# jinhojsk515/spmm

Hardware: AMD Instinct MI355X
Metric: pretrain molecules/sec (higher is better)
Workload: dtype bf16; 1 GPU; SPMM pretrain step, text 12 layers (fusion at 6) + PV 6 layers, H=768, 12 heads, queue 36864, train mode (dropout 0.1), fwd+bwd+clip+AdamW+EMA; global_batch=128, seq_len=128, parallelism=dp1, schedule=eager launches on three HIP streams, packed text rows

## Files before the change

include/spmm_hip.h:

```cpp
#ifndef SPMM_HIP_H
#define SPMM_HIP_H

#include <stdint.h>

#ifdef __HIPCC__
#include <hip/hip_runtime.h>
typedef hipStream_t spmm_stream_t;
#else
typedef void* spmm_stream_t;
#endif

#ifdef __cplusplus
extern "C" {
#endif

int spmm_version(void);
const char* spmm_last_error(void);

#define SPMM_EPI_BF16 0
#define SPMM_EPI_GELU 1
#define SPMM_EPI_F32 2
#define SPMM_EPI_F32_ATOMIC 3
#define SPMM_EPI_GELU_GRAD 4
#define SPMM_EPI_F32_ACC 5
#define SPMM_EPI_GELU_DERIV 6
#define SPMM_EPI_MUL 7

#define SPMM_GEMM_AUTO 0
#define SPMM_GEMM_K128 1
#define SPMM_GEMM_K256x128 2
#define SPMM_GEMM_K256 3
#define SPMM_GEMM_K128PC 5
#define SPMM_GEMM_K256P8 8
#define SPMM_GEMM_K256P8_TILES 9
#define SPMM_GEMM_AUTO_TILES 16
int spmm_gemm_nt(const void* A, long lda, const void* W, long ldw, int M, int N, int K, int splits, const float* bias,
                 const float* div_ptr, float alpha, const void* R, long ldr, const void* G, long ldg, void* C, long ldc,
                 void* C2, long ldc2, int epi, float* colsum, int kernel, const int* M_dev, spmm_stream_t stream);
long spmm_gemm_tn_workspace_bytes(int M, int N, int K, int splits);
int spmm_gemm_tn_splits(int M, int N, int K, int kernel);
int spmm_gemm_tn(const void* A, long lda, const void* B, long ldb, int M, int N, int K, int splits, float alpha, float* C,
                 long ldc, float* workspace, int kernel, const int* M_dev, spmm_stream_t stream);
int spmm_gemm_tn_reduce(const float* ws, int ns, int N, int K, float* C, long ldc, spmm_stream_t stream);
int spmm_colsum_bf16(const void* x, long ld, int R, int C, float* out, const int* R_dev, spmm_stream_t stream);

int spmm_attn_fwd(const void* Q, long ldq, const void* K, long ldk, const void* V, long ldv, const int* kmask,
                  const int* kv_seq, const int* q_row0, const int* q_len, const int* kv_row0, const int* kv_len, void* O,
                  long ldo, float* LSE, int nseq, int nH, int Lq, int Lkv, int causal_from, int is_cross, float dropout_p,
                  const uint64_t* seed_ptr, uint64_t seed_salt, int q_off, int kv_off, spmm_stream_t stream);
int spmm_attn_bwd(const void* Q, long ldq, const void* K, long ldk, const void* V, long ldv, const int* kmask,
                  const int* kv_seq, const int* q_row0, const int* q_len, const int* kv_row0, const int* kv_len,
                  const void* O, long ldo, const float* LSE, const void* dO, long lddo, void* dQ,
                  long lddq, void* dK, long lddk, void* dV, long lddv, int nseq, int nH, int Lq, int Lkv, int causal_from,
                  int is_cross, float dropout_p, const uint64_t* seed_ptr, uint64_t seed_salt, int q_off, int kv_off, int d_mode,
                  float* Dbuf, spmm_stream_t stream);

int spmm_xattn_supported(int H, int nH, int Lq, int Lkv);
int spmm_xattn_pack_wo(const void* W, long ldw, void* out, int H, spmm_stream_t stream);
int spmm_xattn_fwd(const void* Q, long ldq, const void* K, long ldk, const void* V, long ldv, const int* kmask,
                   const int* kv_seq, const int* q_row0, const int* q_len, const int* kv_row0, const int* kv_len,
                   const void* WoF, const float* bo, const void* R, long ldr, const float* gamma, const float* beta, float eps,
                   void* Y, long ldy, void* Z, long ldz, float* mean, float* rstd, void* CTX, long ldc, float* LSE,
                   int nseq, int nH, int Lq, int Lkv, float attn_dropout_p, uint64_t salt_a, float hidden_dropout_p,
                   uint64_t salt_h, const uint64_t* seed_ptr, long row_base, spmm_stream_t stream);
int spmm_segment_sum_bf16(const void* src, const int* start, const int* list, void* out, int U, long W, spmm_stream_t stream);

int spmm_ln_fwd(const void* x, const void* res, const float* gamma, const float* beta, void* y, void* zout, float* mean,
                float* rstd, long rows, int H, float eps, float dropout_p, const uint64_t* seed_ptr, uint64_t salt,
                const int* rows_dev, spmm_stream_t stream);
int spmm_ln_fwd_r32(const void* x, const float* res32, const float* gamma, const float* beta, void* y, float* y32, void* zout,
                    float* mean, float* rstd, long rows, int H, float eps, float dropout_p, const uint64_t* seed_ptr,
                    uint64_t salt, spmm_stream_t stream);
int spmm_ln_bwd(const void* dy, const void* dy2, const void* z, const float* mean, const float* rstd, const float* gamma,
                void* dz, void* dx, float* dgamma, float* dbeta, long rows, int H, float dropout_p,
                const uint64_t* seed_ptr, uint64_t salt, int drop_on_dy, float* dxsum, const int* rows_dev,
                const float* beta_from_y, spmm_stream_t stream);

int spmm_embed_step_ln_fwd(const int* ids, int pos_index, const int* pos_ptr, const float* word, const float* pos, const float* type0,
                           const float* gamma, const float* beta, void* y, long rows, int H, float eps, spmm_stream_t stream);

int spmm_decode_attn(const void* q, long ldq, const void* K, const void* V, long seq_stride, long tok_stride, long head_stride, const int* anc,
                     int anc_ld, int kv_div, int group, void* out, long ldo, int R, int nH, int Lkv, float scale,
                     const int* t_ptr, const void* knew, const void* vnew, long ldn, const int* rowmap, spmm_stream_t stream);

int spmm_decode_xattn(const void* q, long ldq, const void* K, const void* V, long ldkv, const int* kv_seq, const int* kv_row0,
                      const int* kv_len, int group, void* out, long ldo, int R, int nH, int Lkv_max, float scale, spmm_stream_t stream);

int spmm_beam_step(const float* logits, long ldl, int N, int k, int V, int Lmax, int F, int t, const int* t_ptr, int t_off,
                   int* tokens, float* cur_p, float* fin_p, int* fin_len, int* fin_tok, int* fin_n, unsigned char* done,
                   int* anc, int anc_ld, int* ids_out, int* parent_out, int* n_done, const int* mol, const int* rowmap,
                   spmm_stream_t stream);

int spmm_beam_step_until(const float* logits, long ldl, int N, int k, int V, int Lmax, int F, int t, const int* t_ptr, int t_off,
                         int* tokens, float* cur_p, float* fin_p, int* fin_len, int* fin_tok, int* fin_n, unsigned char* done,
                         int* anc, int anc_ld, int* ids_out, int* parent_out, int* n_done, const int* mol, const int* rowmap,
                         int need, spmm_stream_t stream);

int spmm_beam_step_sampled(const float* logits, long ldl, int N, int k, int V, int Lmax, int F, int t, const int* t_ptr, int t_off,
                           int* tokens, float* cur_p, float* fin_p, int* fin_len, int* fin_tok, int* fin_n, unsigned char* done,
                           int* anc, int anc_ld, int* ids_out, int* parent_out, int* n_done, const int* mol, const int* rowmap,
                           const float* noise, long ldn, spmm_stream_t stream);

int spmm_gumbel_noise(const uint64_t* seed_ptr, uint64_t salt, int N, int k, int V, int Lmax, int t, const int* t_ptr, int t_off,
                      const int* mol, long mol_base, float* out, long ldo, spmm_stream_t stream);

int spmm_logit_warp(const float* lc, const float* lu, long ld, int R, int V, float w, float temperature, int top_k, float top_p,
                    int min_keep, float* out, long ldo, spmm_stream_t stream);

#define SPMM_SYNTAX_MASKED (-1e30f)
int spmm_smiles_mask(float* logits, float* logits2, long ld, int R, int V, const int* tokens, long tok_ld, int hist_rows, int k,
                     const int* mol, int Lmax, int t, const int* t_ptr, int t_off, int t_last, const int* table, int* state_out,
                     spmm_stream_t stream);

int spmm_kv_prefill(const void* K, const void* V, long ld, long src_rows, const int* row0, const int* len, const int* dst_row, int E,
                    void* Kc, void* Vc, int R, int nH, int Lmax, spmm_stream_t stream);

int spmm_embed_ln_fwd(int mode, const int* ids, const float* word, const float* pos, const float* type0, const float* pv_x,
// ... 83 lines not shown
```

spmm_amd/csrc/gemm.hip:

```cpp
#include "common.h"
#include "../../include/spmm_hip.h"

namespace {

constexpr int BM = 128, BN = 128, BK = 64;
constexpr int TILE_BYTES = BM * BK * 2;
constexpr int STAGE_BYTES = 2 * TILE_BYTES;

enum Epi { EPI_BF16 = 0, EPI_GELU = 1, EPI_F32 = 2, EPI_F32_ATOMIC = 3, EPI_GELU_GRAD = 4, EPI_F32_ACC = 5, EPI_GELU_DERIV = 6, EPI_MUL = 7 };
constexpr bool epi_is_bf16(int e) { return e == EPI_BF16 || e == EPI_GELU || e == EPI_GELU_GRAD || e == EPI_GELU_DERIV || e == EPI_MUL; }

struct GemmP {
  const bf16* A; long lda;
  const bf16* W; long ldw;
  int M, N, K;
  int ksplit;
  const float* bias;
  const float* div_ptr;
  float alpha;
  const bf16* R; long ldr;
  const bf16* G; long ldg;
  void* C; long ldc;
  bf16* C2; long ldc2;
  float* colsum;
// ... 589 lines not shown
  {
    const int b = blockIdx.x, q = nt >> 3, r = nt & 7, xcd = b & 7, i = b >> 3;
    if (i >= (xcd < r ? q + 1 : q)) return;
    t = (xcd < r ? xcd * (q + 1) : r * (q + 1) + (xcd - r) * q) + i;
  }
  int tile_m, tile_n;
  tile_of(t, ntm, ntn, p.order, tile_m, tile_n);
  const int m0 = tile_m * BM3, n0 = tile_n * BN3;
  const int nk = p.K / BK;

  f32x16 acc[2][2][2];
#pragma unroll
  for (int h = 0; h < 2; ++h)
#pragma unroll
    for (int i = 0; i < 2; ++i)
#pragma unroll
      for (int j = 0; j < 2; ++j)
#pragma unroll
        for (int r = 0; r < 16; ++r) acc[h][i][j][r] = 0.f;

#define STAGE3(kt_)                                                                           \
  do {                                                                                        \
    char* b_ = smem3 + ((kt_) & 1) * STAGE3_BYTES;                                            \
    stage2_dma(p.A, p.lda, m0, p.M, (kt_) * BK, b_, tid, 4);                                  \
    stage2_dma(p.W, p.ldw, n0, p.N, (kt_) * BK, b_ + T3_BYTES, tid, 4);                       \
  } while (0)

  STAGE3(0);
  for (int kt = 0; kt < nk; ++kt) {
    __syncthreads();
    if (kt + 1 < nk) STAGE3(kt + 1);
    const char* As = smem3 + (kt & 1) * STAGE3_BYTES;
    const char* Ws = As + T3_BYTES;
#pragma unroll
    for (int kk = 0; kk < 4; ++kk) {
      const int s = kk * 2 + (lane >> 5);
      bf16x8 af[4], wf[2];
#pragma unroll
      for (int i = 0; i < 4; ++i) {
        const int ar = wm * 128 + i * 32 + (lane & 31);
        af[i] = *(const bf16x8*)(As + ar * 128 + ((s ^ ((ar >> 1) & 7)) << 4));
      }
#pragma unroll
      for (int i = 0; i < 2; ++i) {
        const int wr = wn * 64 + i * 32 + (lane & 31);
        wf[i] = *(const bf16x8*)(Ws + wr * 128 + ((s ^ ((wr >> 1) & 7)) << 4));
      }
#pragma unroll
      for (int h = 0; h < 2; ++h)
#pragma unroll
        for (int ni = 0; ni < 2; ++ni)
#pragma unroll
          for (int mi = 0; mi < 2; ++mi)
            acc[h][ni][mi] = __builtin_amdgcn_mfma_f32_32x32x16_bf16(wf[ni], af[h * 2 + mi], acc[h][ni][mi], 0, 0, 0);
    }
  }
#undef STAGE3
  __syncthreads();
  char* wt = smem3 + wave * 16384;
  float cs_carry[8] = {0.f, 0.f, 0.f, 0.f, 0.f, 0.f, 0.f, 0.f};
#pragma unroll
  for (int h = 0; h < 2; ++h)
    epilogue_bf16<EPI>(p, acc[h], wt, m0 + wm * 128 + h * 64, n0 + wn * 64, lane, cs_carry, h == 1);
}

constexpr int P8_HT = 128 * BK * 2;
constexpr int P8_BUF = 4 * P8_HT;
constexpr int P8_LDS = 2 * P8_BUF;
constexpr int P8_XLDS = 8 * 4096;

template <int OFF>
__device__ __forceinline__ void p8_dsr(bf16x8& d, uint32_t addr) {
  asm volatile("ds_read_b128 %0, %1 offset:%2" : "=v"(d) : "v"(addr), "n"(OFF) : "memory");
}

struct P8Out { uint32_t d[4]; };
__device__ __forceinline__ uint32_t p8_pack2(float a, float b) {
  typedef __bf16 bf16x2 __attribute__((ext_vector_type(2)));
  bf16x2 v; v[0] = (bf16)a; v[1] = (bf16)b;
  return __builtin_bit_cast(uint32_t, v);
}
__device__ __forceinline__ float p8_lo(uint32_t w) { return __builtin_bit_cast(float, w << 16); }
__device__ __forceinline__ float p8_hi(uint32_t w) { return __builtin_bit_cast(float, w & 0xffff0000u); }
typedef uint32_t u32x2 __attribute__((ext_vector_type(2)));
typedef uint32_t u32x4 __attribute__((ext_vector_type(4)));
template <int OFF>
__device__ __forceinline__ void p8_dsw64(uint32_t addr, uint32_t a, uint32_t b) {
  u32x2 v = {a, b};
  asm volatile("ds_write_b64 %0, %1 offset:%2" :: "v"(addr), "v"(v), "n"(OFF) : "memory");
}
template <int OFF>
__device__ __forceinline__ void p8_dsr128u(u32x4& d, uint32_t addr) {
  asm volatile("ds_read_b128 %0, %1 offset:%2" : "=v"(d) : "v"(addr), "n"(OFF) : "memory");
}

template <int EPI, bool INTERIOR, bool HAS_EX, typename Hook>
__device__ __forceinline__ void p8_epilogue_blocks(const GemmP& p, f32x4 (&acc)[2][4][4], uint32_t xb ,
                                                   int m_base, int n_base, int lane, Hook hook) {
  float scale = p.alpha;
  if (p.div_ptr) scale /= *p.div_ptr;
  const int m = lane & 15, g = lane >> 4, r8 = lane >> 3, c16 = lane & 7;
  f32x4 b[4];
#pragma unroll
  for (int ni = 0; ni < 4; ++ni) b[ni] = f32x4{0.f, 0.f, 0.f, 0.f};
  if (p.bias) {
#pragma unroll
    for (int ni = 0; ni < 4; ++ni)
      if (INTERIOR || n_base + ni * 16 + 4 * g < p.N) b[ni] = *(const f32x4*)(p.bias + n_base + ni * 16 + 4 * g);
  }
  uint32_t wad[4];
#pragma unroll
  for (int ni = 0; ni < 4; ++ni) wad[ni] = xb + (uint32_t)(m * 128 + ((((ni * 2 + (g >> 1)) ^ (m & 7)) << 4) | ((g & 1) << 3)));
  const uint32_t rad = xb + (uint32_t)(r8 * 128 + ((c16 ^ (r8 & 7)) << 4));
  const long n = n_base + c16 * 8;
  const bool n_ok = INTERIOR || n < p.N;
  const long row0 = m_base + r8;
  bf16* cp = (bf16*)p.C + row0 * p.ldc + n;
  constexpr bool GELU2 = EPI == EPI_GELU || EPI == EPI_GELU_DERIV;
  constexpr bool DERIV = EPI == EPI_GELU_DERIV;
  constexpr bool MULG = EPI == EPI_MUL;
  bf16* c2p = GELU2 && p.C2 ? p.C2 + row0 * p.ldc2 + n : nullptr;
  u32x4 ex[8];
  const bf16* esrc = (EPI == EPI_GELU_GRAD || MULG) ? p.G : p.R;
  const long eld = (EPI == EPI_GELU_GRAD || MULG) ? p.ldg : p.ldr;
  const long nn = n_ok ? n : 0;
#define P8_EX_LOAD1(I_, R_)                                                                                            \
  do {                                                                                                                 \
    ex[I_] = *(const u32x4*)(esrc + (R_) * eld + nn);                                                                  \
  } while (0)
#define P8_LOAD_EX(H)                                                          \
  if constexpr (HAS_EX) {                                                      \
    _Pragma("unroll") for (int i_ = 0; i_ < 8; ++i_) {                         \
      long r_ = row0 + (H) * 64 + i_ * 8;                                      \
      if (!INTERIOR) r_ = r_ < p.M ? r_ : p.M - 1;                             \
      P8_EX_LOAD1(i_, r_);                                                     \
    }                                                                          \
  }
  P8_LOAD_EX(0);
  float cs[8] = {0.f, 0.f, 0.f, 0.f, 0.f, 0.f, 0.f, 0.f};
#pragma unroll
  for (int h = 0; h < 2; ++h)
#pragma unroll
    for (int mi = 0; mi < 4; ++mi) {
      const int blk = h * 4 + mi;
      const uint32_t bo = (blk & 1) * 2048;
      const bool ok1 = INTERIOR || (n_ok && row0 + blk * 16 < p.M), ok2 = INTERIOR || (n_ok && row0 + blk * 16 + 8 < p.M);
      float v[4][4];
#pragma unroll
      for (int ni = 0; ni < 4; ++ni)
#pragma unroll
        for (int j = 0; j < 4; ++j) v[ni][j] = acc[h][mi][ni][j] * scale + b[ni][j];
#pragma unroll
      for (int ni = 0; ni < 4; ++ni) acc[h][mi][ni] = f32x4{0.f, 0.f, 0.f, 0.f};
      u32x4 o1, o2;
      if constexpr (GELU2) {
        float w[4][4];
#pragma unroll
        for (int ni = 0; ni < 4; ++ni)
#pragma unroll
          for (int j = 0; j < 4; j += 2) {
            const f32x2 x = {v[ni][j], v[ni][j + 1]};
            f32x2 gg, dd = x;
            gelu_erf_pair<DERIV>(x, gg, dd);
            v[ni][j] = gg.x; v[ni][j + 1] = gg.y;
            w[ni][j] = dd.x; w[ni][j + 1] = dd.y;
          }
        if (c2p) {
          u32x4 q1, q2;
#pragma unroll
          for (int ni = 0; ni < 4; ++ni) p8_dsw64<0>(wad[ni] + bo, p8_pack2(w[ni][0], w[ni][1]), p8_pack2(w[ni][2], w[ni][3]));
#pragma unroll
          for (int ni = 0; ni < 4; ++ni) p8_dsw64<0>(wad[ni] + (bo ^ 2048u), p8_pack2(v[ni][0], v[ni][1]), p8_pack2(v[ni][2], v[ni][3]));
          p8_dsr128u<0>(q1, rad + bo);
          p8_dsr128u<1024>(q2, rad + bo);
          p8_dsr128u<0>(o1, rad + (bo ^ 2048u));
          p8_dsr128u<1024>(o2, rad + (bo ^ 2048u));
          asm volatile("s_waitcnt lgkmcnt(0)" ::: "memory");
          __builtin_amdgcn_sched_barrier(0);
          if (ok1) *(u32x4*)(c2p + (long)blk * 16 * p.ldc2) = q1;
          if (ok2) *(u32x4*)(c2p + (long)blk * 16 * p.ldc2 + 8 * p.ldc2) = q2;
        }
      }
      if (!(GELU2 && c2p)) {
#pragma unroll
        for (int ni = 0; ni < 4; ++ni) p8_dsw64<0>(wad[ni] + bo, p8_pack2(v[ni][0], v[ni][1]), p8_pack2(v[ni][2], v[ni][3]));
        p8_dsr128u<0>(o1, rad + bo);
        p8_dsr128u<1024>(o2, rad + bo);
        asm volatile("s_waitcnt lgkmcnt(0)" ::: "memory");
        __builtin_amdgcn_sched_barrier(0);
      }
      if constexpr (EPI == EPI_BF16 && HAS_EX) {
#pragma unroll
        for (int d = 0; d < 4; ++d) {
          o1[d] = p8_pack2(p8_lo(o1[d]) + p8_lo(ex[2 * mi][d]), p8_hi(o1[d]) + p8_hi(ex[2 * mi][d]));
          o2[d] = p8_pack2(p8_lo(o2[d]) + p8_lo(ex[2 * mi + 1][d]), p8_hi(o2[d]) + p8_hi(ex[2 * mi + 1][d]));
        }
      }
      if constexpr (EPI == EPI_GELU_GRAD) {
#pragma unroll
        for (int d = 0; d < 4; ++d) {
          o1[d] = p8_pack2(p8_lo(o1[d]) * gelu_erf_grad(p8_lo(ex[2 * mi][d])), p8_hi(o1[d]) * gelu_erf_grad(p8_hi(ex[2 * mi][d])));
          o2[d] = p8_pack2(p8_lo(o2[d]) * gelu_erf_grad(p8_lo(ex[2 * mi + 1][d])), p8_hi(o2[d]) * gelu_erf_grad(p8_hi(ex[2 * mi + 1][d])));
        }
      }
      if constexpr (EPI == EPI_MUL) {
#pragma unroll
        for (int d = 0; d < 4; ++d) {
          o1[d] = p8_pack2(p8_lo(o1[d]) * p8_lo(ex[2 * mi][d]), p8_hi(o1[d]) * p8_hi(ex[2 * mi][d]));
          o2[d] = p8_pack2(p8_lo(o2[d]) * p8_lo(ex[2 * mi + 1][d]), p8_hi(o2[d]) * p8_hi(ex[2 * mi + 1][d]));
        }
      }
      if constexpr (!GELU2) {
        if (p.colsum) {
#pragma unroll
          for (int d = 0; d < 4; ++d) {
            if (ok1) { cs[2 * d] += p8_lo(o1[d]); cs[2 * d + 1] += p8_hi(o1[d]); }
            if (ok2) { cs[2 * d] += p8_lo(o2[d]); cs[2 * d + 1] += p8_hi(o2[d]); }
          }
        }
      }
#ifdef P8_NOSTORE
      if (p.M < 0) {
#endif
#ifdef P8_STORE_POLICY
      if (ok1) asm volatile("global_store_dwordx4 %0, %1, off " P8_STORE_POLICY :: "v"(cp + (long)blk * 16 * p.ldc), "v"(o1) : "memory");
      if (ok2) asm volatile("global_store_dwordx4 %0, %1, off " P8_STORE_POLICY :: "v"(cp + (long)blk * 16 * p.ldc + 8 * p.ldc), "v"(o2) : "memory");
#else
      if (ok1) *(u32x4*)(cp + (long)blk * 16 * p.ldc) = o1;
      if (ok2) *(u32x4*)(cp + (long)blk * 16 * p.ldc + 8 * p.ldc) = o2;
#endif
#ifdef P8_NOSTORE
      }
#endif
      hook(blk);
      if constexpr (HAS_EX && EPI == EPI_GELU_GRAD) {
        if (blk == 3) { P8_LOAD_EX(1); }
      } else if constexpr (HAS_EX) {
        if (h == 0) {
#pragma unroll
          for (int i_ = 2 * mi; i_ < 2 * mi + 2; ++i_) {
            long r_ = row0 + 64 + i_ * 8;
            if (!INTERIOR) r_ = r_ < p.M ? r_ : p.M - 1;
            P8_EX_LOAD1(i_, r_);
          }
        }
      }
    }
#undef P8_LOAD_EX
#undef P8_EX_LOAD1
  if constexpr (!GELU2) {
    if (p.colsum) {
#pragma unroll
      for (int e = 0; e < 8; ++e) {
        float t = cs[e];
        t += __shfl_xor(t, 8, 64);
        t += __shfl_xor(t, 16, 64);
        t += __shfl_xor(t, 32, 64);
        cs[e] = t;
      }
      if (lane < 8 && n_ok) {
#pragma unroll
        for (int e = 0; e < 8; ++e) atomicAdd(p.colsum + n + e, cs[e]);
      }
    }
  }
}

template <int EPI>
__global__ __launch_bounds__(512) void gemm_nt_p8_kernel(GemmP p) {
  extern __shared__ __attribute__((aligned(16))) char smem8[];
  const int tid = threadIdx.x, lane = tid & 63;
  const int wave = __builtin_amdgcn_readfirstlane(tid >> 6);
  const int wr = wave >> 2, wc = wave & 3;
  GEMM_DYN_M(p);
  const int ntm = (p.M + BM3 - 1) / BM3, ntn = (p.N + BN3 - 1) / BN3, nt = ntm * ntn;
  if ((int)blockIdx.x >= nt) return;
  const int nk = p.K / BK;

  f32x4 acc[2][4][4];
#define P8_ZERO()                                                              \
  _Pragma("unroll") for (int h_ = 0; h_ < 2; ++h_)                             \
  _Pragma("unroll") for (int i_ = 0; i_ < 4; ++i_)                             \
  _Pragma("unroll") for (int j_ = 0; j_ < 4; ++j_) acc[h_][i_][j_] = f32x4{0.f, 0.f, 0.f, 0.f}
  P8_ZERO();

  uint32_t offA[2][2], offW[2][2];
  const uint32_t ls16 = (uint32_t)(((tid & 7) ^ ((tid >> 4) & 7)) * 16);
  int m0, n0;
#define P8_TILE(VB)                                                                                           \
  do {                                                                                                        \
    const int b_ = (VB), q_ = nt >> 3, r_ = nt & 7, xcd_ = b_ & 7, i_ = b_ >> 3;                              \
    const int t_ = (xcd_ < r_ ? xcd_ * (q_ + 1) : r_ * (q_ + 1) + (xcd_ - r_) * q_) + i_;                     \
    int tm_, tn_;                                                                                             \
    tile_of(t_, ntm, ntn, p.order, tm_, tn_);                                                                 \
    m0 = tm_ * BM3; n0 = tn_ * BN3;                                                                           \
    _Pragma("unroll") for (int h_ = 0; h_ < 2; ++h_)                                                          \
    _Pragma("unroll") for (int j_ = 0; j_ < 2; ++j_) {                                                        \
      int row_ = m0 + j_ * 128 + h_ * 64 + (tid >> 3);                                                        \
      row_ = row_ < p.M ? row_ : p.M - 1;                     \
      offA[h_][j_] = (uint32_t)row_ * (uint32_t)(p.lda * 2) + ls16;                                                      \
      int col_ = n0 + (j_ * 2 + (tid >> 8)) * 64 + h_ * 32 + ((tid >> 3) & 31);                               \
      col_ = col_ < p.N ? col_ : p.N - 1;                                                                     \
      offW[h_][j_] = (uint32_t)col_ * (uint32_t)(p.ldw * 2) + ls16;                                                      \
    }                                                                                                         \
  } while (0)
  const char* gA = (const char*)p.A;
  const char* gW = (const char*)p.W;
  const uint32_t lds0 = (uint32_t)(uintptr_t)(LDS_AS char*)smem8;
#define P8_STG(GB, O, SLOT)                                                                                               \
  do {                                                                                                                    \
    const uint32_t d_ = lds0 + (SLOT) + wave * 1024;                                                                      \
    asm volatile("s_mov_b32 m0, %2\n\ts_nop 0\n\tglobal_load_lds_dwordx4 %0, %1" :: "v"((O)[0]), "s"(GB), "s"(d_) : "memory", "m0");          \
    asm volatile("s_mov_b32 m0, %2\n\ts_nop 0\n\tglobal_load_lds_dwordx4 %0, %1" :: "v"((O)[1]), "s"(GB), "s"(d_ + 8192) : "memory", "m0");   \
  } while (0)
#define P8_STG_A(H, BUF, KT) P8_STG((const char*)(gA + (size_t)(KT) * (BK * 2)), offA[H], (BUF) * P8_BUF + (H) * P8_HT)
#define P8_STG_W(H, BUF, KT) P8_STG((const char*)(gW + (size_t)(KT) * (BK * 2)), offW[H], (BUF) * P8_BUF + (2 + (H)) * P8_HT)
#define P8_PROLOGUE()                                                                        \
  do {                                                                                       \
    P8_STG_A(0, 0, 0); P8_STG_W(0, 0, 0); P8_STG_W(1, 0, 0); P8_STG_A(1, 0, 0);              \
    P8_STG_W(0, 1, 1); P8_STG_A(0, 1, 1); P8_STG_W(1, 1, 1);                                 \
  } while (0)

  uint32_t aad[2][2], wad[2][2];
  {
    const uint32_t sw = (uint32_t)((lane >> 1) & 7), r16 = (uint32_t)(lane & 15), q = (uint32_t)(lane >> 4);
#pragma unroll
    for (int kk = 0; kk < 2; ++kk) {
      const uint32_t slot = ((((uint32_t)kk * 4 + q) ^ sw) << 4);
      aad[0][kk] = lds0 + ((uint32_t)wr * 64 + r16) * 128 + slot;
      wad[0][kk] = lds0 + 2 * P8_HT + ((uint32_t)wc * 32 + r16) * 128 + slot;
      aad[1][kk] = aad[0][kk] + P8_BUF;
      wad[1][kk] = wad[0][kk] + P8_BUF;
    }
  }
  bf16x8 fa[4][2], fw0[2][2], fw1[2][2];
#define P8_RD_A(BUF, H)                                                                       \
  do {                                                                                        \
    p8_dsr<(H) * P8_HT + 0 * 2048>(fa[0][0], aad[BUF][0]);                                    \
    p8_dsr<(H) * P8_HT + 1 * 2048>(fa[1][0], aad[BUF][0]);                                    \
    p8_dsr<(H) * P8_HT + 2 * 2048>(fa[2][0], aad[BUF][0]);                                    \
    p8_dsr<(H) * P8_HT + 3 * 2048>(fa[3][0], aad[BUF][0]);                                    \
    p8_dsr<(H) * P8_HT + 0 * 2048>(fa[0][1], aad[BUF][1]);                                    \
    p8_dsr<(H) * P8_HT + 1 * 2048>(fa[1][1], aad[BUF][1]);                                    \
    p8_dsr<(H) * P8_HT + 2 * 2048>(fa[2][1], aad[BUF][1]);                                    \
    p8_dsr<(H) * P8_HT + 3 * 2048>(fa[3][1], aad[BUF][1]);                                    \
  } while (0)
#define P8_RD_W(BUF, H, FW)                                                                   \
  do {                                                                                        \
    p8_dsr<(H) * P8_HT + 0 * 2048>(FW[0][0], wad[BUF][0]);                                    \
    p8_dsr<(H) * P8_HT + 1 * 2048>(FW[1][0], wad[BUF][0]);                                    \
    p8_dsr<(H) * P8_HT + 0 * 2048>(FW[0][1], wad[BUF][1]);                                    \
    p8_dsr<(H) * P8_HT + 1 * 2048>(FW[1][1], wad[BUF][1]);                                    \
  } while (0)
#define P8_MM(H, NH, FW)                                                                                        \
  do {                                                                                                          \
    _Pragma("unroll") for (int kk_ = 0; kk_ < 2; ++kk_)                                                         \
    _Pragma("unroll") for (int mi_ = 0; mi_ < 4; ++mi_)                                                         \
    _Pragma("unroll") for (int ni_ = 0; ni_ < 2; ++ni_)                                                         \
      acc[H][mi_][(NH) * 2 + ni_] =                                                                             \
          __builtin_amdgcn_mfma_f32_16x16x32_bf16(FW[ni_][kk_], fa[mi_][kk_], acc[H][mi_][(NH) * 2 + ni_], 0, 0, 0); \
  } while (0)
#define P8_BAR() __builtin_amdgcn_s_barrier()
#define P8_SB() __builtin_amdgcn_sched_barrier(0)
#define P8_LGKM0() asm volatile("s_waitcnt lgkmcnt(0)" ::: "memory")
#define P8_COMPUTE(H, NH, FW)                    \
  do {                                           \
    P8_BAR();                                    \
    P8_LGKM0();                                  \
    P8_SB();                                     \
    __builtin_amdgcn_s_setprio(1);               \
    P8_MM(H, NH, FW);                            \
    __builtin_amdgcn_s_setprio(0);               \
    P8_SB();                                     \
    P8_BAR();                                    \
    P8_SB();                                     \
  } while (0)

#ifdef P8_PROFILE
  unsigned long long* prof = (unsigned long long*)p.colsum + (size_t)blockIdx.x * 16 * 8;
  p.colsum = nullptr;
  int prof_i = 0;
#define P8_STAMP(K) do { if (prof && tid == 0 && prof_i < 16) prof[prof_i * 8 + (K)] = __builtin_readcyclecounter(); } while (0)
#else
#define P8_STAMP(K) do { } while (0)
#endif
  int vb = blockIdx.x;
  bool pre = false;
  P8_TILE(vb);
  P8_PROLOGUE();
  asm volatile("s_waitcnt vmcnt(6)" ::: "memory");
  P8_BAR();
  P8_SB();
  if (wr == 1) P8_BAR();
  for (;;) {
    P8_STAMP(0);
    const int cm0 = m0, cn0 = n0;
    const int vbn = vb + (int)gridDim.x;
    const bool has_next = vbn < nt;
    const bool pre_next = has_next && cm0 + BM3 <= p.M && cn0 + BN3 <= p.N;
    for (int kt = 0; kt < nk; kt += 2) {
      const bool last = kt + 2 >= nk;
      const bool more = !last || has_next;
      int kn = kt + 2;
      P8_RD_W(0, 0, fw0); P8_SB(); P8_RD_A(0, 0);
      if (!(pre && kt == 0)) P8_STG_A(1, 1, kt + 1);
      asm volatile("s_waitcnt lgkmcnt(8)" ::: "memory");
      P8_COMPUTE(0, 0, fw0);
      if (last && has_next) { P8_TILE(vbn); kn = 0; }
      P8_RD_W(0, 1, fw1);
      if (more) P8_STG_W(0, 0, kn);
      P8_COMPUTE(0, 1, fw1);
      P8_RD_A(0, 1);
      if (more) P8_STG_A(0, 0, kn);
      P8_COMPUTE(1, 1, fw1);
      if (more) {
        P8_STG_W(1, 0, kn);
        if (pre && kt == 0) asm volatile("s_waitcnt vmcnt(22)" ::: "memory");
        else asm volatile("s_waitcnt vmcnt(6)" ::: "memory");
      } else {
        asm volatile("s_waitcnt vmcnt(0)" ::: "memory");
      }
      P8_COMPUTE(1, 0, fw0);
      P8_RD_W(1, 0, fw0); P8_SB(); P8_RD_A(1, 0);
      if (more) P8_STG_A(1, 0, kn);
      asm volatile("s_waitcnt lgkmcnt(8)" ::: "memory");
      P8_COMPUTE(0, 0, fw0);
      P8_RD_W(1, 1, fw1);
      if (more) P8_STG_W(0, 1, kn + 1);
      P8_COMPUTE(0, 1, fw1);
      P8_RD_A(1, 1);
      if (more) P8_STG_A(0, 1, kn + 1);
      P8_COMPUTE(1, 1, fw1);
      if (more) {
        P8_STG_W(1, 1, kn + 1);
        if (last && pre_next) {
          P8_STG_A(1, 1, kn + 1);
          asm volatile("s_waitcnt vmcnt(8)" ::: "memory");
        } else {
          asm volatile("s_waitcnt vmcnt(6)" ::: "memory");
        }
      }
      P8_COMPUTE(1, 0, fw0);
    }
    P8_STAMP(2);

    if (wr == 0) P8_BAR();
    P8_SB();
    {
      int lane_e = lane;
      asm volatile("" : "+v"(lane_e));
      GemmP q = p;
      asm volatile("" : "+s"(q.C), "+s"(q.ldc), "+s"(q.C2), "+s"(q.ldc2));
      asm volatile("" : "+s"(q.R), "+s"(q.ldr), "+s"(q.G), "+s"(q.ldg));
      asm volatile("" : "+s"(q.bias), "+s"(q.colsum), "+s"(q.div_ptr), "+s"(q.alpha), "+s"(q.M), "+s"(q.N));
      auto hook = [](int) {};
      const uint32_t xb = lds0 + P8_LDS + wave * 4096;
      const int mb = cm0 + wr * 128, nb = cn0 + wc * 64;
      const bool interior = cm0 + BM3 <= q.M && cn0 + BN3 <= q.N;
      if constexpr (EPI == EPI_GELU_GRAD || EPI == EPI_MUL) {
        if (interior) p8_epilogue_blocks<EPI, true, true>(q, acc, xb, mb, nb, lane_e, hook);
        else p8_epilogue_blocks<EPI, false, true>(q, acc, xb, mb, nb, lane_e, hook);
      } else if (EPI == EPI_BF16 && q.R != nullptr) {
        if (interior) p8_epilogue_blocks<EPI, true, true>(q, acc, xb, mb, nb, lane_e, hook);
        else p8_epilogue_blocks<EPI, false, true>(q, acc, xb, mb, nb, lane_e, hook);
      } else {
        if (interior) p8_epilogue_blocks<EPI, true, false>(q, acc, xb, mb, nb, lane_e, hook);
        else p8_epilogue_blocks<EPI, false, false>(q, acc, xb, mb, nb, lane_e, hook);
      }
    }
    P8_SB();
    if (wr == 1) P8_BAR();
    P8_STAMP(4);
#ifdef P8_PROFILE
    ++prof_i;
#endif
    if (!has_next) break;
    vb = vbn;
    pre = pre_next;
    P8_SB();
  }
  if (wr == 0) P8_BAR();
#undef P8_ZERO
#undef P8_STAMP
#undef P8_TILE
#undef P8_PROLOGUE
#undef P8_STG
#undef P8_STG_A
#undef P8_STG_W
#undef P8_RD_A
#undef P8_RD_W
#undef P8_MM
#undef P8_COMPUTE
#undef P8_BAR
#undef P8_SB
#undef P8_LGKM0
}

template <typename K>
int raise_lds(K kernel, int bytes, const char* what) {
  hipError_t e = hipFuncSetAttribute((const void*)kernel, hipFuncAttributeMaxDynamicSharedMemorySize, bytes);
  if (e != hipSuccess) {
    spmm_set_error("spmm_gemm_nt: cannot raise the dynamic LDS of %s to %d: %s", what, bytes, hipGetErrorString(e));
    return SPMM_ERR_LAUNCH;
  }
  return SPMM_OK;
}

template <int EPI>
int launch_p8_one(const GemmP& p, hipStream_t st, bool persist) {
  static const int rc = raise_lds(gemm_nt_p8_kernel<EPI>, P8_LDS + P8_XLDS, "the 8-phase kernel");
  if (rc != SPMM_OK) return rc;
  const int nt = ((p.M + BM3 - 1) / BM3) * ((p.N + BN3 - 1) / BN3);
  static const int ncu = [] { int dev = 0, n = 0; (void)hipGetDevice(&dev); (void)hipDeviceGetAttribute(&n, hipDeviceAttributeMultiprocessorCount, dev); return n > 0 ? n & ~7 : 256; }();
  dim3 grid(persist && nt > ncu ? ncu : nt);
  hipLaunchKernelGGL((gemm_nt_p8_kernel<EPI>), grid, dim3(512), P8_LDS + P8_XLDS, st, p);
  return SPMM_OK;
}
int launch_p8(int epi, const GemmP& p, hipStream_t st, bool persist) {
  switch (epi) {
    case EPI_BF16: return launch_p8_one<EPI_BF16>(p, st, persist);
    case EPI_GELU: return launch_p8_one<EPI_GELU>(p, st, persist);
    case EPI_GELU_GRAD: return launch_p8_one<EPI_GELU_GRAD>(p, st, persist);
    case EPI_GELU_DERIV: return launch_p8_one<EPI_GELU_DERIV>(p, st, persist);
    case EPI_MUL: return launch_p8_one<EPI_MUL>(p, st, persist);
    default: return -1;
  }
}

template <int EPI>
int launch_v3_one(const GemmP& p, hipStream_t st) {
  static const int rc = raise_lds(gemm_nt_v3_kernel<EPI>, LDS3_BYTES, "the 256x256 kernel");
  if (rc != SPMM_OK) return rc;
  dim3 grid(((p.M + BM3 - 1) / BM3) * ((p.N + BN3 - 1) / BN3));
  hipLaunchKernelGGL((gemm_nt_v3_kernel<EPI>), grid, dim3(512), LDS3_BYTES, st, p);
  return SPMM_OK;
}
int launch_v3(int epi, const GemmP& p, hipStream_t st) {
  switch (epi) {
    case EPI_BF16: return launch_v3_one<EPI_BF16>(p, st);
    case EPI_GELU: return launch_v3_one<EPI_GELU>(p, st);
    case EPI_GELU_GRAD: return launch_v3_one<EPI_GELU_GRAD>(p, st);
    case EPI_GELU_DERIV: return launch_v3_one<EPI_GELU_DERIV>(p, st);
    case EPI_MUL: return launch_v3_one<EPI_MUL>(p, st);
    default: return -1;
  }
}

template <int EPI>
int launch_v2_one(const GemmP& p, hipStream_t st) {
  static const int rc = raise_lds(gemm_nt_v2_kernel<EPI>, LDS2_BYTES, "the 256x128 kernel");
  if (rc != SPMM_OK) return rc;
  dim3 grid(((p.M + BM2 - 1) / BM2) * ((p.N + BN - 1) / BN));
  hipLaunchKernelGGL((gemm_nt_v2_kernel<EPI>), grid, dim3(512), LDS2_BYTES, st, p);
  return SPMM_OK;
}
int launch_v2(int epi, const GemmP& p, hipStream_t st) {
  switch (epi) {
    case EPI_BF16: return launch_v2_one<EPI_BF16>(p, st);
    case EPI_GELU: return launch_v2_one<EPI_GELU>(p, st);
    case EPI_F32: return launch_v2_one<EPI_F32>(p, st);
    case EPI_GELU_GRAD: return launch_v2_one<EPI_GELU_GRAD>(p, st);
    case EPI_GELU_DERIV: return launch_v2_one<EPI_GELU_DERIV>(p, st);
    case EPI_MUL: return launch_v2_one<EPI_MUL>(p, st);
    case EPI_F32_ACC: return launch_v2_one<EPI_F32_ACC>(p, st);
    default: return -1;
  }
}

template <typename K>
int pc_attr(K kernel) {
  static const hipError_t e = hipFuncSetAttribute((const void*)kernel, hipFuncAttributeMaxDynamicSharedMemorySize, PC_LDS);
  return e == hipSuccess ? 0 : 1;
}
#define PC_LAUNCH(E)                                                                                   \
  case E:                                                                                              \
    if (pc_attr(gemm_nt_pc_kernel<E>)) { spmm_set_error("spmm_gemm_nt: cannot raise the LDS limit of the loader/compute kernel"); return SPMM_ERR_LAUNCH; } \
    hipLaunchKernelGGL((gemm_nt_pc_kernel<E>), grid, dim3(PC_THREADS), PC_LDS, st, p);                        \
    break
int launch_pc(int epi, const GemmP& p, dim3 grid, hipStream_t st) {
  switch (epi) {
    PC_LAUNCH(EPI_BF16); PC_LAUNCH(EPI_GELU); PC_LAUNCH(EPI_F32); PC_LAUNCH(EPI_F32_ATOMIC); PC_LAUNCH(EPI_GELU_GRAD); PC_LAUNCH(EPI_F32_ACC);
    PC_LAUNCH(EPI_GELU_DERIV); PC_LAUNCH(EPI_MUL);
    default: return -1;
  }
  return 0;
}
#undef PC_LAUNCH

int launch_v1(int epi, const GemmP& p, dim3 grid, hipStream_t st) {
  switch (epi) {
    case EPI_BF16: hipLaunchKernelGGL((gemm_nt_kernel<EPI_BF16>), grid, dim3(256), 0, st, p); break;
    case EPI_GELU: hipLaunchKernelGGL((gemm_nt_kernel<EPI_GELU>), grid, dim3(256), 0, st, p); break;
    case EPI_F32: hipLaunchKernelGGL((gemm_nt_kernel<EPI_F32>), grid, dim3(256), 0, st, p); break;
    case EPI_F32_ATOMIC: hipLaunchKernelGGL((gemm_nt_kernel<EPI_F32_ATOMIC>), grid, dim3(256), 0, st, p); break;
    case EPI_GELU_GRAD: hipLaunchKernelGGL((gemm_nt_kernel<EPI_GELU_GRAD>), grid, dim3(256), 0, st, p); break;
    case EPI_F32_ACC: hipLaunchKernelGGL((gemm_nt_kernel<EPI_F32_ACC>), grid, dim3(256), 0, st, p); break;
    case EPI_GELU_DERIV: hipLaunchKernelGGL((gemm_nt_kernel<EPI_GELU_DERIV>), grid, dim3(256), 0, st, p); break;
    case EPI_MUL: hipLaunchKernelGGL((gemm_nt_kernel<EPI_MUL>), grid, dim3(256), 0, st, p); break;
    default: return -1;
  }
  return SPMM_OK;
}

inline bool is_bf16_epi(int epi) { return epi_is_bf16(epi); }
inline bool p8_ok(const GemmP& p, int epi) {
  return is_bf16_epi(epi) && p.K % 128 == 0 && p.N % 8 == 0 && (unsigned long)p.M * (unsigned long)p.lda * 2ul < (1ul << 32) &&
         (unsigned long)p.N * (unsigned long)p.ldw * 2ul < (1ul << 32);
}

int pick_tile(int M, int N, int epi) {
  const bool bf = is_bf16_epi(epi);
  if (M >= 6000) {
    const long t3 = (long)((M + 255) / 256) * ((N + 255) / 256);
    if (bf && t3 >= 96) return 3;
    return (epi != EPI_F32_ATOMIC) ? 2 : 1;
  }
  auto tiles = [&](int bm, int bn) { return (double)((M + bm - 1) / bm) * ((N + bn - 1) / bn); };
  auto fill = [](double t) { const double w = (double)(long)((t + 255) / 256); return t / (256.0 * w); };
  const double t3 = tiles(256, 256), t2 = tiles(256, 128), t1 = tiles(128, 128);
  const double s3 = bf ? 1.20 * fill(t3) : 0.0;
  const double s2 = (M >= 512 && epi != EPI_F32_ATOMIC) ? 0.85 * fill(t2) : 0.0;
  const double s1 = 0.80 * (t1 < 256 ? t1 / 256.0 : 1.0);
  if (s3 >= s2 && s3 >= s1) return 3;
  return s2 >= s1 ? 2 : 1;
}

}

extern "C" int spmm_gemm_nt(const void* A, long lda, const void* W, long ldw, int M, int N, int K, int splits,
                            const float* bias, const float* div_ptr, float alpha, const void* R, long ldr,
                            const void* G, long ldg, void* C, long ldc, void* C2, long ldc2, int epi, float* colsum,
                            int kernel, const int* M_dev, hipStream_t stream) {
  SPMM_CHECK_SHAPE(M > 0 && N > 0 && K > 0, "spmm_gemm_nt: empty problem M=%d N=%d K=%d", M, N, K);
  SPMM_CHECK_SHAPE(K % 64 == 0, "spmm_gemm_nt: K=%d must be a multiple of 64", K);
  SPMM_CHECK_SHAPE(N % 4 == 0, "spmm_gemm_nt: N=%d must be a multiple of 4", N);
  SPMM_CHECK_SHAPE(lda % 8 == 0 && ldw % 8 == 0, "spmm_gemm_nt: lda/ldw must be multiples of 8 elements");
  SPMM_CHECK_SHAPE(ldc % 4 == 0, "spmm_gemm_nt: ldc must be a multiple of 4");
  SPMM_CHECK_SHAPE(!is_bf16_epi(epi) || (ldc % 8 == 0 && (!R || ldr % 8 == 0) && (!G || ldg % 8 == 0) && (!C2 || ldc2 % 8 == 0) && (uintptr_t)C % 16 == 0),
                   "spmm_gemm_nt: bf16 outputs need 16-B aligned rows (ldc/ldr/ldg/ldc2 multiples of 8)");
  SPMM_CHECK_SHAPE(is_bf16_epi(epi) || !R || (ldr % 4 == 0 && (uintptr_t)R % 8 == 0),
                   "spmm_gemm_nt: R of an fp32-output epilogue is read 4 columns at a time (ldr a multiple of 4, R 8-B aligned)");
  SPMM_CHECK_SHAPE(((uintptr_t)A % 16 == 0) && ((uintptr_t)W % 16 == 0), "spmm_gemm_nt: A/W must be 16-B aligned");
  SPMM_CHECK_SHAPE(epi >= EPI_BF16 && epi <= EPI_MUL, "spmm_gemm_nt: unknown epilogue %d", epi);
  if (splits < 1) splits = 1;
  SPMM_CHECK_SHAPE(splits == 1 || epi == EPI_F32_ATOMIC, "spmm_gemm_nt: split-K needs the atomic epilogue");
  SPMM_CHECK_SHAPE((epi != EPI_GELU_GRAD && epi != EPI_MUL) || G != nullptr, "spmm_gemm_nt: the GELU-grad / multiply epilogues need G");
  SPMM_CHECK_SHAPE(colsum == nullptr || epi == EPI_BF16 || epi == EPI_GELU_GRAD || epi == EPI_MUL, "spmm_gemm_nt: colsum is only fused into the bf16 / GELU-grad / multiply epilogues");
  int ksplit = ((K / 64 + splits - 1) / splits) * 64;
  splits = (K + ksplit - 1) / ksplit;
  GemmP p;
  p.A = (const bf16*)A; p.lda = lda; p.W = (const bf16*)W; p.ldw = ldw;
  p.M = M; p.N = N; p.K = K; p.ksplit = ksplit; p.bias = bias; p.div_ptr = div_ptr; p.alpha = alpha;
  p.R = (const bf16*)R; p.ldr = ldr; p.G = (const bf16*)G; p.ldg = ldg; p.C = C; p.ldc = ldc;
  p.C2 = (bf16*)C2; p.ldc2 = ldc2; p.colsum = colsum;
  p.M_ptr = nullptr;
  p.order = K > 1024 ? 0 : 2;

  int k = kernel == SPMM_GEMM_AUTO_TILES ? 0 : kernel;
  if (k == 0) {
    const int tile = splits > 1 ? 1 : pick_tile(M, N, epi);
    k = tile == 3 ? (p8_ok(p, epi) ? (kernel == SPMM_GEMM_AUTO_TILES ? 9 : 8) : 3) : tile;
    if (k == 2 && (epi == EPI_F32_ATOMIC || M < 512)) k = 1;
  }
  const bool pc_fits = (unsigned long)p.M * (unsigned long)p.lda * 2ul < (1ul << 32) && (unsigned long)p.N * (unsigned long)p.ldw * 2ul < (1ul << 32);
  const long t128 = (long)((M + BM - 1) / BM) * ((N + BN - 1) / BN) * splits;
  if (k == 1 && kernel != 1 && pc_fits && PC_AUTO && t128 <= 256 && ksplit >= 4 * BK) k = 5;
  SPMM_CHECK_SHAPE(k == 1 || k == 2 || k == 3 || k == 5 || k == 8 || k == 9, "spmm_gemm_nt: unknown kernel selector %d", kernel);
  SPMM_CHECK_SHAPE(k != 5 || pc_fits, "spmm_gemm_nt: kernel 5 addresses its operands with 32-bit byte offsets (< 4 GiB each)");
  SPMM_CHECK_SHAPE((k != 8 && k != 9) || p8_ok(p, epi), "spmm_gemm_nt: the 8-phase kernel needs a bf16-output epilogue, K %% 128 == 0, N %% 8 == 0 and operands < 4 GiB");
  SPMM_CHECK_SHAPE(k != 3 || is_bf16_epi(epi), "spmm_gemm_nt: the 256x256 kernel has bf16-output epilogues only");
  SPMM_CHECK_SHAPE(k != 2 || epi != EPI_F32_ATOMIC, "spmm_gemm_nt: the 256x128 kernel has no atomic epilogue");
  SPMM_CHECK_SHAPE(k == 1 || k == 5 || splits == 1, "spmm_gemm_nt: split-K runs on the 128x128 kernels only");
  p.M_ptr = M_dev;
  int rc;
  if (k == 8 || k == 9) rc = launch_p8(epi, p, stream, k == 8);
  else if (k == 3) rc = launch_v3(epi, p, stream);
  else if (k == 2) rc = launch_v2(epi, p, stream);
  else if (k == 5) rc = launch_pc(epi, p, dim3(((M + BM - 1) / BM) * ((N + BN - 1) / BN), 1, splits), stream);
  else rc = launch_v1(epi, p, dim3(((M + BM - 1) / BM) * ((N + BN - 1) / BN), 1, splits), stream);
  if (rc > 0) return rc;
  if (rc < 0) { spmm_set_error("spmm_gemm_nt: epilogue %d is not built for kernel %d", epi, k); return SPMM_ERR_UNSUPPORTED; }
  SPMM_LAUNCH_CHECK("spmm_gemm_nt");
  return SPMM_OK;
}
```

Measured before the change: 2444 molecules/s.

## Route large fp32-accumulate GEMMs to the 256x256 8-phase kernel

Adds an fp32 accumulate-into-C epilogue (EPI_F32_ACC, with optional bf16 residual) to the 8-phase 256x256 kernel, using an LDS transpose so C is read and written in coalesced 16-byte chunks. Auto-selection now sends large-M F32_ACC GEMMs with enough tiles to this kernel instead of the 256x128 kernel. It also packs the bf16 add and multiply epilogues and the colsum accumulation into two-wide float vectors. The goal is higher MMA tile reuse for residual-accumulating GEMMs. The costs are extra C read traffic in the epilogue, a changed vmcnt wait, and more register pressure.

```diff
diff --git a/include/spmm_hip.h b/include/spmm_hip.h
--- a/include/spmm_hip.h
+++ b/include/spmm_hip.h
@@ -33,6 +33,8 @@
 #define SPMM_GEMM_K128PC 5
 #define SPMM_GEMM_K256P8 8
 #define SPMM_GEMM_K256P8_TILES 9
+#define SPMM_GEMM_K256P8_F32 10
+#define SPMM_GEMM_K256P8_F32_TILES 11
 #define SPMM_GEMM_AUTO_TILES 16
 int spmm_gemm_nt(const void* A, long lda, const void* W, long ldw, int M, int N, int K, int splits, const float* bias,
                  const float* div_ptr, float alpha, const void* R, long ldr, const void* G, long ldg, void* C, long ldc,
diff --git a/spmm_amd/csrc/gemm.hip b/spmm_amd/csrc/gemm.hip
--- a/spmm_amd/csrc/gemm.hip
+++ b/spmm_amd/csrc/gemm.hip
@@ -695,6 +695,8 @@
 }
 __device__ __forceinline__ float p8_lo(uint32_t w) { return __builtin_bit_cast(float, w << 16); }
 __device__ __forceinline__ float p8_hi(uint32_t w) { return __builtin_bit_cast(float, w & 0xffff0000u); }
+__device__ __forceinline__ f32x2 p8_unpack(uint32_t w) { return f32x2{p8_lo(w), p8_hi(w)}; }
+__device__ __forceinline__ uint32_t p8_pack(f32x2 v) { return p8_pack2(v.x, v.y); }
 typedef uint32_t u32x2 __attribute__((ext_vector_type(2)));
 typedef uint32_t u32x4 __attribute__((ext_vector_type(4)));
 template <int OFF>
@@ -750,7 +752,7 @@
     }                                                                          \
   }
   P8_LOAD_EX(0);
-  float cs[8] = {0.f, 0.f, 0.f, 0.f, 0.f, 0.f, 0.f, 0.f};
+  f32x2 cs[4] = {f32x2{0.f, 0.f}, f32x2{0.f, 0.f}, f32x2{0.f, 0.f}, f32x2{0.f, 0.f}};
 #pragma unroll
   for (int h = 0; h < 2; ++h)
 #pragma unroll
@@ -805,8 +807,8 @@
       if constexpr (EPI == EPI_BF16 && HAS_EX) {
 #pragma unroll
         for (int d = 0; d < 4; ++d) {
-          o1[d] = p8_pack2(p8_lo(o1[d]) + p8_lo(ex[2 * mi][d]), p8_hi(o1[d]) + p8_hi(ex[2 * mi][d]));
-          o2[d] = p8_pack2(p8_lo(o2[d]) + p8_lo(ex[2 * mi + 1][d]), p8_hi(o2[d]) + p8_hi(ex[2 * mi + 1][d]));
+          o1[d] = p8_pack(p8_unpack(o1[d]) + p8_unpack(ex[2 * mi][d]));
+          o2[d] = p8_pack(p8_unpack(o2[d]) + p8_unpack(ex[2 * mi + 1][d]));
         }
       }
       if constexpr (EPI == EPI_GELU_GRAD) {
@@ -819,16 +821,21 @@
       if constexpr (EPI == EPI_MUL) {
 #pragma unroll
         for (int d = 0; d < 4; ++d) {
-          o1[d] = p8_pack2(p8_lo(o1[d]) * p8_lo(ex[2 * mi][d]), p8_hi(o1[d]) * p8_hi(ex[2 * mi][d]));
-          o2[d] = p8_pack2(p8_lo(o2[d]) * p8_lo(ex[2 * mi + 1][d]), p8_hi(o2[d]) * p8_hi(ex[2 * mi + 1][d]));
+          o1[d] = p8_pack(p8_unpack(o1[d]) * p8_unpack(ex[2 * mi][d]));
+          o2[d] = p8_pack(p8_unpack(o2[d]) * p8_unpack(ex[2 * mi + 1][d]));
         }
       }
       if constexpr (!GELU2) {
         if (p.colsum) {
 #pragma unroll
           for (int d = 0; d < 4; ++d) {
-            if (ok1) { cs[2 * d] += p8_lo(o1[d]); cs[2 * d + 1] += p8_hi(o1[d]); }
-            if (ok2) { cs[2 * d] += p8_lo(o2[d]); cs[2 * d + 1] += p8_hi(o2[d]); }
+            if constexpr (EPI == EPI_GELU_GRAD) {
+              if (ok1) { cs[d].x += p8_lo(o1[d]); cs[d].y += p8_hi(o1[d]); }
+              if (ok2) { cs[d].x += p8_lo(o2[d]); cs[d].y += p8_hi(o2[d]); }
+            } else {
+              if (ok1) cs[d] += p8_unpack(o1[d]);
+              if (ok2) cs[d] += p8_unpack(o2[d]);
+            }
           }
         }
       }
@@ -865,18 +872,91 @@
     if (p.colsum) {
 #pragma unroll
       for (int e = 0; e < 8; ++e) {
-        float t = cs[e];
+        float t = cs[e >> 1][e & 1];
         t += __shfl_xor(t, 8, 64);
         t += __shfl_xor(t, 16, 64);
         t += __shfl_xor(t, 32, 64);
-        cs[e] = t;
+        cs[e >> 1][e & 1] = t;
       }
       if (lane < 8 && n_ok) {
 #pragma unroll
-        for (int e = 0; e < 8; ++e) atomicAdd(p.colsum + n + e, cs[e]);
-      }
-    }
-  }
+        for (int e = 0; e < 8; ++e) atomicAdd(p.colsum + n + e, cs[e >> 1][e & 1]);
+      }
+    }
+  }
+}
+
+template <bool INTERIOR, bool HAS_R>
+__device__ __forceinline__ void p8_epilogue_f32acc(const GemmP& p, f32x4 (&acc)[2][4][4], uint32_t xb, int m_base, int n_base, int lane) {
+  float scale = p.alpha;
+  if (p.div_ptr) scale /= *p.div_ptr;
+  const int m = lane & 15, g = lane >> 4;
+  f32x4 b[4];
+#pragma unroll
+  for (int ni = 0; ni < 4; ++ni) b[ni] = f32x4{0.f, 0.f, 0.f, 0.f};
+  if (p.bias) {
+#pragma unroll
+    for (int ni = 0; ni < 4; ++ni)
+      if (INTERIOR || n_base + ni * 16 + 4 * g < p.N) b[ni] = *(const f32x4*)(p.bias + n_base + ni * 16 + 4 * g);
+  }
+  const long arow0 = m_base + m;
+  long acol[4];
+#pragma unroll
+  for (int ni = 0; ni < 4; ++ni) { const long n_ = n_base + ni * 16 + 4 * g; acol[ni] = (INTERIOR || n_ < p.N) ? n_ : 0; }
+  const int r4 = lane >> 4, c16 = lane & 15;
+  uint32_t wad[4], rad[4];
+#pragma unroll
+  for (int ni = 0; ni < 4; ++ni) wad[ni] = xb + (uint32_t)(m * 256 + (((ni * 4 + g) ^ m) << 4));
+#pragma unroll
+  for (int i = 0; i < 4; ++i) rad[i] = xb + (uint32_t)((4 * i + r4) * 256 + ((c16 ^ (4 * i + r4)) << 4));
+  const long crow0 = m_base + r4;
+  const long cn = n_base + 4 * c16;
+  const bool c_ok = INTERIOR || cn < p.N;
+  const long ccol = c_ok ? cn : 0;
+  float* const C = (float*)p.C;
+#pragma unroll
+  for (int h = 0; h < 2; ++h)
+#pragma unroll
+    for (int mi = 0; mi < 4; ++mi) {
+      const int blk = h * 4 + mi;
+      f32x4 cin[4];
+      u32x2 rin[4];
+#pragma unroll
+      for (int i = 0; i < 4; ++i) {
+        long r_ = crow0 + blk * 16 + 4 * i;
+        if (!INTERIOR) r_ = r_ < p.M ? r_ : p.M - 1;
+        cin[i] = *(const f32x4*)(C + r_ * p.ldc + ccol);
+      }
+      if constexpr (HAS_R) {
+        long r_ = arow0 + blk * 16;
+        if (!INTERIOR) r_ = r_ < p.M ? r_ : p.M - 1;
+#pragma unroll
+        for (int ni = 0; ni < 4; ++ni) rin[ni] = *(const u32x2*)(p.R + r_ * p.ldr + acol[ni]);
+      }
+      f32x4 v[4];
+#pragma unroll
+      for (int ni = 0; ni < 4; ++ni) {
+#pragma unroll
+        for (int j = 0; j < 4; ++j) v[ni][j] = acc[h][mi][ni][j] * scale + b[ni][j];
+        acc[h][mi][ni] = f32x4{0.f, 0.f, 0.f, 0.f};
+        if constexpr (HAS_R) {
+          v[ni][0] += p8_lo(rin[ni][0]); v[ni][1] += p8_hi(rin[ni][0]);
+          v[ni][2] += p8_lo(rin[ni][1]); v[ni][3] += p8_hi(rin[ni][1]);
+        }
+      }
+#pragma unroll
+      for (int ni = 0; ni < 4; ++ni) asm volatile("ds_write_b128 %0, %1" :: "v"(wad[ni]), "v"(v[ni]) : "memory");
+#pragma unroll
+      for (int i = 0; i < 4; ++i) asm volatile("ds_read_b128 %0, %1" : "=v"(v[i]) : "v"(rad[i]) : "memory");
+      asm volatile("s_waitcnt lgkmcnt(0)" ::: "memory");
+      __builtin_amdgcn_sched_barrier(0);
+#pragma unroll
+      for (int i = 0; i < 4; ++i) {
+        const long r_ = crow0 + blk * 16 + 4 * i;
+        const f32x4 o = cin[i] + v[i];
+        if (INTERIOR || (c_ok && r_ < p.M)) *(f32x4*)(C + r_ * p.ldc + ccol) = o;
+      }
+    }
 }
 
 template <int EPI>
@@ -1028,8 +1108,10 @@
       P8_COMPUTE(1, 1, fw1);
       if (more) {
         P8_STG_W(1, 0, kn);
-        if (pre && kt == 0) asm volatile("s_waitcnt vmcnt(22)" ::: "memory");
-        else asm volatile("s_waitcnt vmcnt(6)" ::: "memory");
+        if (pre && kt == 0) {
+          if constexpr (EPI == EPI_F32_ACC) asm volatile("s_waitcnt vmcnt(63)" ::: "memory");
+          else asm volatile("s_waitcnt vmcnt(22)" ::: "memory");
+        } else asm volatile("s_waitcnt vmcnt(6)" ::: "memory");
       } else {
         asm volatile("s_waitcnt vmcnt(0)" ::: "memory");
       }
@@ -1070,7 +1152,15 @@
       const uint32_t xb = lds0 + P8_LDS + wave * 4096;
       const int mb = cm0 + wr * 128, nb = cn0 + wc * 64;
       const bool interior = cm0 + BM3 <= q.M && cn0 + BN3 <= q.N;
-      if constexpr (EPI == EPI_GELU_GRAD || EPI == EPI_MUL) {
+      if constexpr (EPI == EPI_F32_ACC) {
+        if (q.R != nullptr) {
+          if (interior) p8_epilogue_f32acc<true, true>(q, acc, xb, mb, nb, lane_e);
+          else p8_epilogue_f32acc<false, true>(q, acc, xb, mb, nb, lane_e);
+        } else {
+          if (interior) p8_epilogue_f32acc<true, false>(q, acc, xb, mb, nb, lane_e);
+          else p8_epilogue_f32acc<false, false>(q, acc, xb, mb, nb, lane_e);
+        }
+      } else if constexpr (EPI == EPI_GELU_GRAD || EPI == EPI_MUL) {
         if (interior) p8_epilogue_blocks<EPI, true, true>(q, acc, xb, mb, nb, lane_e, hook);
         else p8_epilogue_blocks<EPI, false, true>(q, acc, xb, mb, nb, lane_e, hook);
       } else if (EPI == EPI_BF16 && q.R != nullptr) {
@@ -1136,6 +1226,7 @@
     case EPI_GELU_GRAD: return launch_p8_one<EPI_GELU_GRAD>(p, st, persist);
     case EPI_GELU_DERIV: return launch_p8_one<EPI_GELU_DERIV>(p, st, persist);
     case EPI_MUL: return launch_p8_one<EPI_MUL>(p, st, persist);
+    case EPI_F32_ACC: return launch_p8_one<EPI_F32_ACC>(p, st, persist);
     default: return -1;
   }
 }
@@ -1216,10 +1307,13 @@
 }
 
 inline bool is_bf16_epi(int epi) { return epi_is_bf16(epi); }
-inline bool p8_ok(const GemmP& p, int epi) {
-  return is_bf16_epi(epi) && p.K % 128 == 0 && p.N % 8 == 0 && (unsigned long)p.M * (unsigned long)p.lda * 2ul < (1ul << 32) &&
+inline bool p8_shape_ok(const GemmP& p) {
+  return p.K % 128 == 0 && p.N % 8 == 0 && (unsigned long)p.M * (unsigned long)p.lda * 2ul < (1ul << 32) &&
          (unsigned long)p.N * (unsigned long)p.ldw * 2ul < (1ul << 32);
 }
+inline bool p8_ok(const GemmP& p, int epi) { return is_bf16_epi(epi) && p8_shape_ok(p); }
+inline bool p8f_ok(const GemmP& p, int epi) { return epi == EPI_F32_ACC && p8_shape_ok(p) && (uintptr_t)p.C % 16 == 0; }
+constexpr long P8F_MIN_TILES = 96;
 
 int pick_tile(int M, int N, int epi) {
   const bool bf = is_bf16_epi(epi);
@@ -1274,19 +1368,22 @@
     const int tile = splits > 1 ? 1 : pick_tile(M, N, epi);
     k = tile == 3 ? (p8_ok(p, epi) ? (kernel == SPMM_GEMM_AUTO_TILES ? 9 : 8) : 3) : tile;
     if (k == 2 && (epi == EPI_F32_ATOMIC || M < 512)) k = 1;
+    if (k == 2 && M >= 6000 && p8f_ok(p, epi) && (long)((M + BM3 - 1) / BM3) * ((N + BN3 - 1) / BN3) >= P8F_MIN_TILES)
+      k = kernel == SPMM_GEMM_AUTO_TILES ? 11 : 10;
   }
   const bool pc_fits = (unsigned long)p.M * (unsigned long)p.lda * 2ul < (1ul << 32) && (unsigned long)p.N * (unsigned long)p.ldw * 2ul < (1ul << 32);
   const long t128 = (long)((M + BM - 1) / BM) * ((N + BN - 1) / BN) * splits;
   if (k == 1 && kernel != 1 && pc_fits && PC_AUTO && t128 <= 256 && ksplit >= 4 * BK) k = 5;
-  SPMM_CHECK_SHAPE(k == 1 || k == 2 || k == 3 || k == 5 || k == 8 || k == 9, "spmm_gemm_nt: unknown kernel selector %d", kernel);
+  SPMM_CHECK_SHAPE(k == 1 || k == 2 || k == 3 || k == 5 || k == 8 || k == 9 || k == 10 || k == 11, "spmm_gemm_nt: unknown kernel selector %d", kernel);
   SPMM_CHECK_SHAPE(k != 5 || pc_fits, "spmm_gemm_nt: kernel 5 addresses its operands with 32-bit byte offsets (< 4 GiB each)");
   SPMM_CHECK_SHAPE((k != 8 && k != 9) || p8_ok(p, epi), "spmm_gemm_nt: the 8-phase kernel needs a bf16-output epilogue, K %% 128 == 0, N %% 8 == 0 and operands < 4 GiB");
+  SPMM_CHECK_SHAPE((k != 10 && k != 11) || p8f_ok(p, epi), "spmm_gemm_nt: the 8-phase kernel's fp32 epilogue is SPMM_EPI_F32_ACC and needs K %% 128 == 0, N %% 8 == 0, a 16-B aligned C and operands < 4 GiB");
   SPMM_CHECK_SHAPE(k != 3 || is_bf16_epi(epi), "spmm_gemm_nt: the 256x256 kernel has bf16-output epilogues only");
   SPMM_CHECK_SHAPE(k != 2 || epi != EPI_F32_ATOMIC, "spmm_gemm_nt: the 256x128 kernel has no atomic epilogue");
   SPMM_CHECK_SHAPE(k == 1 || k == 5 || splits == 1, "spmm_gemm_nt: split-K runs on the 128x128 kernels only");
   p.M_ptr = M_dev;
   int rc;
-  if (k == 8 || k == 9) rc = launch_p8(epi, p, stream, k == 8);
+  if (k == 8 || k == 9 || k == 10 || k == 11) rc = launch_p8(epi, p, stream, k == 8 || k == 10);
   else if (k == 3) rc = launch_v3(epi, p, stream);
   else if (k == 2) rc = launch_v2(epi, p, stream);
   else if (k == 5) rc = launch_pc(epi, p, dim3(((M + BM - 1) / BM) * ((N + BN - 1) / BN), 1, splits), stream);
```

Result: no change. 2453 molecules/s (median of 6 runs) (+0.4%).
